# leoelm/Bayesian_inference_for_NN

Measured on NVIDIA B200. Metric: posterior_grad_evals_per_s, higher is better.
Workload: dtype f32 (tensor-core products on two int8 fixed-point slices per operand, kind::i8, exact int32 accumulate; f32 everywhere else)

## Files before the change

### bayesian_inference_for_nn_b200/csrc/tc_fused.cuh

```cuda
#pragma once
#include "tc_layer2.cuh"

namespace pyb {

constexpr int TF_THREADS = 384;
template <int CP> struct TfCfg {
  static constexpr int STAGES = 5;
  static constexpr int W2_BYTES = 2 * 256 * CP * 4;
  static constexpr int ZX_BYTES = 2 * CP * 128 * 4;
  static constexpr int SMEM = STAGES * TP_STAGE_BYTES + 1024  + 1024  + 2048  +
                              128  + W2_BYTES + ZX_BYTES;
  static constexpr int SMEM_I8 = SMEM + 4096;
};
__device__ __forceinline__ void tc_ld_16x256b_x4_raw(uint32_t taddr, uint32_t* r) {
  asm volatile(
      "tcgen05.ld.sync.aligned.16x256b.x4.b32 "
      "{%0, %1, %2, %3, %4, %5, %6, %7, %8, %9, %10, %11, %12, %13, %14, %15}, [%16];"
      : "=r"(r[0]), "=r"(r[1]), "=r"(r[2]), "=r"(r[3]), "=r"(r[4]), "=r"(r[5]), "=r"(r[6]), "=r"(r[7]), "=r"(r[8]),
        "=r"(r[9]), "=r"(r[10]), "=r"(r[11]), "=r"(r[12]), "=r"(r[13]), "=r"(r[14]), "=r"(r[15])
      : "r"(taddr)
      : "memory");
}
__device__ __forceinline__ void tc_mma_i8_pair(uint32_t tmem_d, uint64_t adesc, uint64_t bdesc, uint32_t idesc,
                                               uint32_t accumulate) {
  asm volatile(
      "{\n"
      ".reg .pred p;\n"
      "setp.ne.b32 p, %4, 0;\n"
      "tcgen05.mma.cta_group::2.kind::i8 [%0], %1, %2, %3, p;\n"
      "}\n" ::"r"(tmem_d),
      "l"(adesc), "l"(bdesc), "r"(idesc), "r"(accumulate)
      : "memory");
}
__device__ __forceinline__ void slice4_i8(const float* d, float zq, uint32_t& hw, uint32_t& lw) {
  constexpr float M = 12582912.0f;
  uint32_t hb[4], lb[4];
#pragma unroll
  for (int r = 0; r < 4; ++r) {
    const float t = fmaf(d[r], zq, M);
    const float h = t - M;
    const float e = fmaf(d[r], zq, -h);
    const float u = fmaf(e, 254.0f, M);
    hb[r] = __float_as_uint(t);
    lb[r] = __float_as_uint(u);
  }
  hw = __byte_perm(__byte_perm(hb[0], hb[1], 0x0040), __byte_perm(hb[2], hb[3], 0x0040), 0x5410);
  lw = __byte_perm(__byte_perm(lb[0], lb[1], 0x0040), __byte_perm(lb[2], lb[3], 0x0040), 0x5410);
}

__device__ __forceinline__ void tc_ld_16x256b_x4(uint32_t taddr, float* v) {
  uint32_t r[16];
  asm volatile(
      "tcgen05.ld.sync.aligned.16x256b.x4.b32 "
      "{%0, %1, %2, %3, %4, %5, %6, %7, %8, %9, %10, %11, %12, %13, %14, %15}, [%16];"
      : "=r"(r[0]), "=r"(r[1]), "=r"(r[2]), "=r"(r[3]), "=r"(r[4]), "=r"(r[5]), "=r"(r[6]), "=r"(r[7]), "=r"(r[8]),
        "=r"(r[9]), "=r"(r[10]), "=r"(r[11]), "=r"(r[12]), "=r"(r[13]), "=r"(r[14]), "=r"(r[15])
      : "r"(taddr)
      : "memory");
#pragma unroll
  for (int i = 0; i < 16; ++i) v[i] = __uint_as_float(r[i]);
}
template <int CP>
__device__ __forceinline__ int w2_slot(int h, int c) {
  return ((((h >> 3) * 2 + (h & 1)) * (CP / 4) + (c >> 2)) * 4 + ((h >> 1) & 3)) * 4 + (c & 3);
}
__device__ __forceinline__ void split_pair(float x0, float x1, uint32_t& hw, uint32_t& lw) {
  const __nv_bfloat162 hp = __floats2bfloat162_rn(x0, x1);
  hw = *reinterpret_cast<const uint32_t*>(&hp);
  const __nv_bfloat162 lp = __floats2bfloat162_rn(x0 - __uint_as_float(hw << 16), x1 - __uint_as_float(hw & 0xffff0000u));
  lw = *reinterpret_cast<const uint32_t*>(&lp);
}

template <int CP, bool FWD, int I8 = 0>
__global__ void __cluster_dims__(2, 1, 1) __launch_bounds__(TF_THREADS, 1)
tc_g1_layer2_fused(const __grid_constant__ CUtensorMap tmA_hi, const __grid_constant__ CUtensorMap tmA_lo,
                   const __grid_constant__ CUtensorMap tmB_hi, const __grid_constant__ CUtensorMap tmB_lo,
                   const TcGemmParams p, const Layer2Params l2) {
  constexpr int STAGES = TfCfg<CP>::STAGES;
  extern __shared__ uint8_t smem_raw[];
  uint8_t* smem = smem_raw + ((1024u - (smem_u32(smem_raw) & 1023u)) & 1023u);
  uint8_t* stage_base = smem;
  uint64_t* bars = (uint64_t*)(smem + STAGES * TP_STAGE_BYTES);
  uint64_t* full_bar = bars;
  uint64_t* empty_bar = bars + STAGES;
  uint64_t* tmem_full = bars + 2 * STAGES;
  uint64_t* tmem_empty = bars + 2 * STAGES + 2;
  uint32_t* tmem_ptr = (uint32_t*)(bars + 2 * STAGES + 4);
  float* bias_s = (float*)(smem + STAGES * TP_STAGE_BYTES + 1024);
  float* b2_s = bias_s + 512;
  float* W2_s = b2_s + 32;
  float* zx_s = W2_s + 2 * 256 * CP;
  float* cw_s = zx_s + 2 * CP * 128;
  float* zq_s = cw_s + 512;

  const int warp = __shfl_sync(0xffffffffu, (int)(threadIdx.x >> 5), 0), lane = threadIdx.x & 31;
  const uint32_t rank = cluster_ctarank();
  const int cluster_id = blockIdx.x >> 1, n_clusters = gridDim.x >> 1;
  constexpr int KSTAGE = I8 ? 64 : TC_BK;
  const int nk = (p.K + KSTAGE - 1) / KSTAGE;
  const int H = p.H;
  const int half_rows = H >> 1;
  const uint32_t cta_bytes = 2 * TC_A_TILE_BYTES + 2 * (uint32_t)half_rows * TC_BK * 2;

  if (warp == 8 && lane == 0) {
    asm volatile("prefetch.tensormap [%0];" ::"l"(&tmA_hi) : "memory");
    asm volatile("prefetch.tensormap [%0];" ::"l"(&tmA_lo) : "memory");
    asm volatile("prefetch.tensormap [%0];" ::"l"(&tmB_hi) : "memory");
    asm volatile("prefetch.tensormap [%0];" ::"l"(&tmB_lo) : "memory");
  }
  if (warp == 9 && lane == 0) {
    for (int s = 0; s < STAGES; ++s) { mbar_init(&full_bar[s], 1); mbar_init(&empty_bar[s], 1); }
    mbar_init(&tmem_full[0], 1); mbar_init(&tmem_full[1], 1);
    mbar_init(&tmem_empty[0], 16); mbar_init(&tmem_empty[1], 16);
    asm volatile("fence.mbarrier_init.release.cluster;" ::: "memory");
  }
  if (warp == 10) {
    asm volatile("tcgen05.alloc.cta_group::2.sync.aligned.shared::cta.b32 [%0], %1;" ::"r"(smem_u32(tmem_ptr)), "r"(512)
                 : "memory");
    asm volatile("tcgen05.relinquish_alloc_permit.cta_group::2.sync.aligned;" ::: "memory");
  }
  tc_fence_before();
  __syncthreads();
  cluster_sync_all();
  tc_fence_after();
  const uint32_t tmem_base = *tmem_ptr;

  if (warp >= 8) {
   asm volatile("setmaxnreg.dec.sync.aligned.u32 40;");
   if (warp == 8) {
    if (lane == 0) {
      int stage = 0;
      uint32_t phase = 0;
      for (int item = cluster_id; item < p.total_items; item += n_clusters) {
        int b, mp, split;
        tc_decode(p, item, b, mp, split);
        const int arow = p.a_row0 + (mp * 2 + (int)rank) * 128;
        const int brow = b * H + (int)rank * half_rows;
        for (int kc = 0; kc < nk; ++kc) {
          (I8 ? mbar_wait_sleep(&empty_bar[stage], phase ^ 1) : mbar_wait(&empty_bar[stage], phase ^ 1));
          uint8_t* st = stage_base + stage * TP_STAGE_BYTES;
          if (rank == 0) mbar_expect_tx(&full_bar[stage], 2 * cta_bytes);
          const int k0 = kc * KSTAGE;
          tma_load_2d_pair(st, &tmA_hi, &full_bar[stage], k0, arow);
          tma_load_2d_pair(st + TC_A_TILE_BYTES, &tmA_lo, &full_bar[stage], k0, arow);
          tma_load_2d_pair(st + 2 * TC_A_TILE_BYTES, &tmB_hi, &full_bar[stage], k0, brow);
          tma_load_2d_pair(st + 2 * TC_A_TILE_BYTES + 8192, &tmB_lo, &full_bar[stage], k0, brow);
          if (++stage == STAGES) { stage = 0; phase ^= 1; }
        }
      }
    }
  } else if (warp == 9) {
    if (rank == 0 && lane == 0) {
      const uint32_t idesc = (I8 ? (2u << 4) : (1u << 4)) | (1u << 7) | (1u << 10) | ((uint32_t)(H >> 3) << 17) | ((256u >> 4) << 24);
      int stage = 0, it = 0;
      uint32_t phase = 0;
      const int k_tail = p.K - (nk - 1) * KSTAGE;
      for (int item = cluster_id; item < p.total_items; item += n_clusters, ++it) {
        const int acc = I8 ? 0 : (it & 1);
        const uint32_t acc_phase = I8 ? (uint32_t)(it & 1) : (uint32_t)((it >> 1) & 1);
        (I8 ? mbar_wait_sleep(&tmem_empty[acc], acc_phase ^ 1) : mbar_wait(&tmem_empty[acc], acc_phase ^ 1));
        tc_fence_after();
        const uint32_t d = tmem_base + (uint32_t)acc * 256;
        for (int kc = 0; kc < nk; ++kc) {
          (I8 ? mbar_wait_sleep(&full_bar[stage], phase) : mbar_wait(&full_bar[stage], phase));
          tc_fence_after();
          const uint32_t st = smem_u32(stage_base + stage * TP_STAGE_BYTES);
          const int nks = (kc == nk - 1 && k_tail <= KSTAGE / 2) ? 1 : 2;
          for (int ks = 0; ks < nks; ++ks) {
            const uint32_t koff = ks * 32;
            const uint64_t ah = make_smem_desc_sw64(st + koff);
            const uint64_t al = make_smem_desc_sw64(st + TC_A_TILE_BYTES + koff);
            const uint64_t bh = make_smem_desc_sw64(st + 2 * TC_A_TILE_BYTES + koff);
            const uint64_t bl = make_smem_desc_sw64(st + 2 * TC_A_TILE_BYTES + 8192 + koff);
            const uint32_t accum = (kc != 0) || (ks != 0);
            if (I8) {
              tc_mma_i8_pair(d, ah, bh, idesc, accum);
              tc_mma_i8_pair(d + 256, ah, bl, idesc, accum);
              tc_mma_i8_pair(d + 256, al, bh, idesc, 1);
            } else {
              tc_mma_bf16_pair(d, ah, bh, idesc, accum);
              tc_mma_bf16_pair(d, al, bh, idesc, 1);
              tc_mma_bf16_pair(d, ah, bl, idesc, 1);
            }
          }
          tc_commit_pair(&empty_bar[stage]);
          if (++stage == STAGES) { stage = 0; phase ^= 1; }
        }
        tc_commit_pair(&tmem_full[acc]);
      }
    }
   }
  } else {
    asm volatile("setmaxnreg.inc.sync.aligned.u32 232;");
    const int half = warp >> 2;
    const int quad = warp & 3;
    const int g = lane >> 2, t = lane & 3;
    const int eall = threadIdx.x;
    const uint32_t lane_addr = (uint32_t)(quad * 32) << 16;
    const int Hh = H >> 1;
    const int C = l2.C;
    const float invN = l2.scale / (float)l2.N;
    const int r_own = 2 * (t & 1) + (t >> 1);
    const int row_own = quad * 32 + g + 8 * r_own;
    const int pos0 = quad * 32 + 4 * g;
    const int hbase = half * Hh + 2 * t;
    uint16_t* z2_hi = reinterpret_cast<uint16_t*>(l2.z2_hi);
    uint16_t* z2_lo = reinterpret_cast<uint16_t*>(l2.z2_lo);
    for (int i = eall; i < 2 * 256 * CP; i += 256) W2_s[i] = 0.f;
    if (eall < 32) b2_s[eall] = 0.f;
    asm volatile("bar.sync 1, 256;" ::: "memory");
    auto fetch_consts = [&](int item, int buf) {
      int b, mp, split;
      tc_decode(p, item, b, mp, split);
      const float* th = l2.theta + (int64_t)b * l2.P;
      if (eall < H) {
        const int h = eall;
        const float* src = th + l2.w2_off + (int64_t)h * C;
        const uint32_t dst = smem_u32(W2_s + buf * 256 * CP + w2_slot<CP>(h, 0));
#pragma unroll
        for (int c = 0; c < CP; ++c)
          if (c < C)
            asm volatile("cp.async.ca.shared.global [%0], [%1], 4;" ::"r"(dst + (uint32_t)(((c >> 2) * 16 + (c & 3)) * 4)),
                         "l"(src + c) : "memory");
        asm volatile("cp.async.ca.shared.global [%0], [%1], 4;" ::"r"(smem_u32(bias_s + buf * 256 + h)),
                     "l"(p.bias + (int64_t)b * p.bias_stride + h) : "memory");
      }
      if (eall < C)
        asm volatile("cp.async.ca.shared.global [%0], [%1], 4;" ::"r"(smem_u32(b2_s + buf * 16 + eall)),
                     "l"(th + l2.b2_off + eall) : "memory");
      if (I8 && eall < H) {
        asm volatile("cp.async.ca.shared.global [%0], [%1], 4;" ::"r"(smem_u32(cw_s + buf * 256 + eall)),
                     "l"(l2.cw + (int64_t)b * H + eall) : "memory");
        if (I8 == 2 && !FWD)
          asm volatile("cp.async.ca.shared.global [%0], [%1], 4;" ::"r"(smem_u32(zq_s + buf * 256 + eall)),
                       "l"(l2.zq + (int64_t)b * H + eall) : "memory");
      }
    };
    if (cluster_id < p.total_items) fetch_consts(cluster_id, 0);
    int it = 0;
    for (int item = cluster_id; item < p.total_items; item += n_clusters, ++it) {
      int b, mp, split;
      tc_decode(p, item, b, mp, split);
      const int mt = mp * 2 + (int)rank;
      const int cbuf = it & 1;
      const int acc = I8 ? 0 : cbuf;
      const uint32_t acc_phase = I8 ? (uint32_t)(it & 1) : (uint32_t)((it >> 1) & 1);
      float* bs = bias_s + cbuf * 256;
      float* b2b = b2_s + cbuf * 16;
      float* W2b = W2_s + cbuf * 256 * CP;
      float sxr[4] = {0.f, 0.f, 0.f, 0.f};
      if (I8) {
#pragma unroll
        for (int r = 0; r < 4; ++r) {
          const int rg = mt * 128 + quad * 32 + g + 8 * r;
          sxr[r] = rg < p.M_valid ? __ldg(l2.sx + rg) : 0.f;
        }
      }
      asm volatile("cp.async.wait_all;" ::: "memory");
      asm volatile("bar.sync 1, 256;" ::: "memory");
      (I8 ? mbar_wait_sleep(&tmem_full[acc], acc_phase) : mbar_wait(&tmem_full[acc], acc_phase));
      tc_fence_after();
      const int64_t blk_w = (((((int64_t)b * p.out_tiles + mt) * H) + hbase) * 128 + pos0) >> 2;
      uint2* pa_hi = reinterpret_cast<uint2*>(p.out_hi) + blk_w;
      uint2* pa_lo = reinterpret_cast<uint2*>(p.out_lo) + blk_w;
      uint2* pz_hi = reinterpret_cast<uint2*>(l2.zt_hi) + blk_w;
      uint2* pz_lo = reinterpret_cast<uint2*>(l2.zt_lo) + blk_w;
      const float4* w4b = reinterpret_cast<const float4*>(W2b) + (((half * Hh) >> 3) * 2 * (CP / 4)) * 4 + t;
      const float* bsb = bs + hbase;
      const float* cwb = cw_s + cbuf * 256 + hbase;
      const float* zqb = zq_s + cbuf * 256 + hbase;
      uint32_t* pzi_hi = nullptr; uint32_t* pzi_lo = nullptr;
      if (I8 == 2 && !FWD) {
        const int64_t blk_b = ((((int64_t)b * p.out_tiles + mt) * H) + hbase) * 128 + pos0;
        pzi_hi = reinterpret_cast<uint32_t*>(l2.zi_hi + blk_b);
        pzi_lo = reinterpret_cast<uint32_t*>(l2.zi_lo + blk_b);
      }
      float2 z[4][CP / 2];
#pragma unroll
      for (int r = 0; r < 4; ++r)
#pragma unroll
        for (int c = 0; c < CP / 2; ++c) z[r][c] = make_float2(0.f, 0.f);
      uint32_t mask[4] = {0u, 0u, 0u, 0u};
#pragma unroll
      for (int ch = 0; ch < 4; ++ch) {
        if (ch * 32 < Hh) {
          const uint32_t col = (uint32_t)(acc * 256 + half * Hh + ch * 32);
          float v[32];
          if (I8) {
#pragma unroll
            for (int hf = 0; hf < 2; ++hf) {
              uint32_t rh[16], rc[16];
              tc_ld_16x256b_x4_raw(tmem_base + lane_addr + ((uint32_t)(16 * hf) << 16) + col, rh);
              tc_ld_16x256b_x4_raw(tmem_base + lane_addr + ((uint32_t)(16 * hf) << 16) + 256u + col, rc);
              asm volatile("tcgen05.wait::ld.sync.aligned;" ::: "memory");
#pragma unroll
              for (int j = 0; j < 16; ++j)
                v[16 * hf + j] = fmaf((float)(int)rc[j], 1.0f / 254.0f, (float)(int)rh[j]);
            }
          } else {
            tc_ld_16x256b_x4(tmem_base + lane_addr + col, v);
            tc_ld_16x256b_x4(tmem_base + lane_addr + (16u << 16) + col, v + 16);
            asm volatile("tcgen05.wait::ld.sync.aligned;" ::: "memory");
          }
          uint32_t m = 0u;
#pragma unroll
          for (int kb = 0; kb < 4; ++kb) {
            const float2 bb = *reinterpret_cast<const float2*>(bsb + ch * 32 + 8 * kb);
            float2 cc = make_float2(0.f, 0.f);
            if (I8) cc = *reinterpret_cast<const float2*>(cwb + ch * 32 + 8 * kb);
            float a[4][2];
#pragma unroll
            for (int r = 0; r < 4; ++r) {
              const float* vv = v + (r >> 1) * 16 + kb * 4 + (r & 1) * 2;
              if (I8) {
                a[r][0] = fmaxf(fmaf(vv[0], sxr[r] * cc.x, bb.x), 0.f);
                a[r][1] = fmaxf(fmaf(vv[1], sxr[r] * cc.y, bb.y), 0.f);
              } else {
                a[r][0] = fmaxf(vv[0] + bb.x, 0.f);
                a[r][1] = fmaxf(vv[1] + bb.y, 0.f);
              }
              if (!FWD) {
                m |= (a[r][0] > 0.f ? 1u : 0u) << (kb * 8 + r * 2);
                m |= (a[r][1] > 0.f ? 1u : 0u) << (kb * 8 + r * 2 + 1);
              }
            }
#pragma unroll
            for (int i = 0; i < 2; ++i) {
              const float4* w4 = w4b + (((ch * 4 + kb) * 2 + i) * (CP / 4)) * 4;
#pragma unroll
              for (int c4 = 0; c4 < CP / 4; ++c4) {
                const float4 w = w4[c4 * 4];
                const float2 w01 = make_float2(w.x, w.y), w23 = make_float2(w.z, w.w);
#pragma unroll
                for (int r = 0; r < 4; ++r) {
                  const float2 aa = make_float2(a[r][i], a[r][i]);
                  z[r][2 * c4] = __ffma2_rn(aa, w01, z[r][2 * c4]);
                  z[r][2 * c4 + 1] = __ffma2_rn(aa, w23, z[r][2 * c4 + 1]);
                }
              }
              if (!FWD) {
                uint32_t hw0, lw0, hw1, lw1;
                split_pair(a[0][i], a[1][i], hw0, lw0);
                split_pair(a[2][i], a[3][i], hw1, lw1);
                const int w_off = (ch * 32 + 8 * kb + i) * 32;
                __stcs(pa_hi + w_off, make_uint2(hw0, hw1));
                __stcs(pa_lo + w_off, make_uint2(lw0, lw1));
              }
            }
          }
          mask[ch] = m;
        }
      }
      tc_fence_before();
      __syncwarp();
      if (lane == 0) mbar_arrive_leader_relaxed(&tmem_empty[acc]);
      if (item + n_clusters < p.total_items) fetch_consts(item + n_clusters, cbuf ^ 1);
      float zo[CP];
      {
        const bool b0 = t & 1, b1 = t & 2;
#pragma unroll
        for (int c = 0; c < CP; ++c) {
          const float z0 = (c & 1) ? z[0][c >> 1].y : z[0][c >> 1].x, z1 = (c & 1) ? z[1][c >> 1].y : z[1][c >> 1].x;
          const float z2v = (c & 1) ? z[2][c >> 1].y : z[2][c >> 1].x, z3 = (c & 1) ? z[3][c >> 1].y : z[3][c >> 1].x;
          float k0 = b0 ? z2v : z0, k1 = b0 ? z3 : z1;
          const float g0 = __shfl_xor_sync(0xffffffffu, b0 ? z0 : z2v, 1);
          const float g1 = __shfl_xor_sync(0xffffffffu, b0 ? z1 : z3, 1);
          k0 = b0 ? g0 + k0 : k0 + g0;
          k1 = b0 ? g1 + k1 : k1 + g1;
          const float kk = b1 ? k1 : k0;
          const float gg = __shfl_xor_sync(0xffffffffu, b1 ? k0 : k1, 2);
          zo[c] = b1 ? gg + kk : kk + gg;
        }
      }
#pragma unroll
      for (int c = 0; c < CP; ++c) zx_s[(half * CP + c) * 128 + row_own] = zo[c];
      asm volatile("bar.sync 2, 256;" ::: "memory");
      float zf[CP], dz[CP];
#pragma unroll
      for (int c = 0; c < CP; ++c) zf[c] = (b2b[c] + zx_s[c * 128 + row_own]) + zx_s[(CP + c) * 128 + row_own];
      const int row_g = mt * 128 + row_own;
      if (FWD) {
        if (half == 0 && row_g < p.M_valid) {
          float* o = l2.fwd_out + ((int64_t)b * l2.N + row_g) * C;
          if (l2.out_act == PYB_ACT_SOFTMAX) {
            float mx = -INFINITY;
#pragma unroll
            for (int c = 0; c < CP; ++c) if (c < C) mx = fmaxf(mx, zf[c]);
            float se = 0.f;
#pragma unroll
            for (int c = 0; c < CP; ++c) if (c < C) se += expf(zf[c] - mx);
            const float inv = 1.0f / se;
#pragma unroll
            for (int c = 0; c < CP; ++c) if (c < C) o[c] = expf(zf[c] - mx) * inv;
          } else {
#pragma unroll
            for (int c = 0; c < CP; ++c) if (c < C) o[c] = act_apply(zf[c], l2.out_act);
          }
        }
        continue;
      }
      float loss_r = 0.f;
      l2_loss_dz<CP>(l2, row_g, row_g < p.M_valid, zf, dz, loss_r, invN);
      if (half == 0) {
        const int64_t blk2 = (((int64_t)b * p.out_tiles + mt) * L2_CMAX) * 128 + pos0 + r_own;
#pragma unroll
        for (int c = 0; c < CP; ++c) {
          __nv_bfloat16 hb, lb;
          split_bf16(dz[c], hb, lb);
          z2_hi[blk2 + c * 128] = __bfloat16_as_ushort(hb);
          z2_lo[blk2 + c * 128] = __bfloat16_as_ushort(lb);
        }
        const int64_t grp = (int64_t)b * l2.n_groups + mt * 4 + quad;
        float mine = 0.f;
#pragma unroll
        for (int c = 0; c < CP; ++c) {
          const float sm = warp_sum(dz[c]);
          if (lane == c) mine = sm;
        }
        if (lane < CP) l2.b2_partial[grp * L2_CMAX + lane] = mine;
        const float ls = warp_sum(loss_r);
        if (lane == 0) l2.loss_partial[grp] = (double)ls;
      }
      float2 dzp[4][CP / 2];
#pragma unroll
      for (int r = 0; r < 4; ++r) {
        const int src = (lane & ~3) | ((r >> 1) | ((r & 1) << 1));
#pragma unroll
        for (int c = 0; c < CP / 2; ++c) {
          dzp[r][c].x = __shfl_sync(0xffffffffu, dz[2 * c], src);
          dzp[r][c].y = __shfl_sync(0xffffffffu, dz[2 * c + 1], src);
        }
      }
#pragma unroll
      for (int ch = 0; ch < 4; ++ch) {
        if (ch * 32 < Hh) {
          const uint32_t m = mask[ch];
#pragma unroll
          for (int kb = 0; kb < 4; ++kb) {
#pragma unroll
            for (int i = 0; i < 2; ++i) {
              const float4* w4 = w4b + (((ch * 4 + kb) * 2 + i) * (CP / 4)) * 4;
              float2 s[4];
#pragma unroll
              for (int r = 0; r < 4; ++r) s[r] = make_float2(0.f, 0.f);
#pragma unroll
              for (int c4 = 0; c4 < CP / 4; ++c4) {
                const float4 w = w4[c4 * 4];
                const float2 w01 = make_float2(w.x, w.y), w23 = make_float2(w.z, w.w);
#pragma unroll
                for (int r = 0; r < 4; ++r) {
                  s[r] = __ffma2_rn(dzp[r][2 * c4], w01, s[r]);
                  s[r] = __ffma2_rn(dzp[r][2 * c4 + 1], w23, s[r]);
                }
              }
              float d[4];
#pragma unroll
              for (int r = 0; r < 4; ++r) d[r] = ((m >> (kb * 8 + r * 2 + i)) & 1u) ? s[r].x + s[r].y : 0.f;
              const int w_off = (ch * 32 + 8 * kb + i) * 32;
              if (I8 == 2) {
                uint32_t hw, lw;
                slice4_i8(d, zqb[ch * 32 + 8 * kb + i], hw, lw);
                __stcs(pzi_hi + w_off, hw);
                __stcs(pzi_lo + w_off, lw);
              } else {
                uint32_t hw0, lw0, hw1, lw1;
                split_pair(d[0], d[1], hw0, lw0);
                split_pair(d[2], d[3], hw1, lw1);
                __stcs(pz_hi + w_off, make_uint2(hw0, hw1));
                __stcs(pz_lo + w_off, make_uint2(lw0, lw1));
              }
            }
          }
        }
      }
    }
  }
  tc_fence_before();
  __syncthreads();
  cluster_sync_all();
  if (warp == 10) {
    tc_fence_after();
    asm volatile("tcgen05.dealloc.cta_group::2.sync.aligned.b32 %0, %1;" ::"r"(tmem_base), "r"(512) : "memory");
  }
}

}
```

### bayesian_inference_for_nn_b200/csrc/tc_layer2.cuh

```cuda
#pragma once
#include "tc_gemm.cuh"

namespace pyb {

__device__ __forceinline__ void split_bf16(float x, __nv_bfloat16& hi, __nv_bfloat16& lo) {
  hi = __float2bfloat16_rn(x);
  lo = __float2bfloat16_rn(x - __bfloat162float(hi));
}

__global__ void k_split_rows(const float* src, int64_t R, int C, int64_t lds, __nv_bfloat16* hi, __nv_bfloat16* lo,
                             int64_t ldd) {
  const int64_t total = R * C;
  for (int64_t i = (int64_t)blockIdx.x * blockDim.x + threadIdx.x; i < total; i += (int64_t)gridDim.x * blockDim.x) {
    int64_t r = i / C;
    int c = (int)(i - r * C);
    __nv_bfloat16 h, l;
    split_bf16(src[r * lds + c], h, l);
    hi[r * ldd + c] = h;
    lo[r * ldd + c] = l;
  }
}
__global__ void k_split_rows2(const float* __restrict__ src, int64_t R, int C2, int64_t lds, __nv_bfloat16* __restrict__ hi,
                              __nv_bfloat16* __restrict__ lo, int64_t ldd) {
  const int64_t total = R * C2;
  for (int64_t i = (int64_t)blockIdx.x * blockDim.x + threadIdx.x; i < total; i += (int64_t)gridDim.x * blockDim.x) {
    const int64_t r = i / C2;
    const int c = 2 * (int)(i - r * C2);
    const float2 v = *reinterpret_cast<const float2*>(src + r * lds + c);
    __nv_bfloat16 h0, l0, h1, l1;
    split_bf16(v.x, h0, l0);
    split_bf16(v.y, h1, l1);
    *reinterpret_cast<__nv_bfloat162*>(hi + r * ldd + c) = __nv_bfloat162(h0, h1);
    *reinterpret_cast<__nv_bfloat162*>(lo + r * ldd + c) = __nv_bfloat162(l0, l1);
  }
}

__host__ __device__ __forceinline__ int fused_row_pos(int r) { return (r & ~31) | ((r & 7) << 2) | ((r >> 3) & 3); }

__global__ void k_split_transpose(const float* src, int64_t sb, int R, int C, int64_t lds, __nv_bfloat16* hi,
                                  __nv_bfloat16* lo, int64_t db, int64_t ldd, int perm = 0) {
  __shared__ float t[32][33];
  const float* s = src + (int64_t)blockIdx.z * sb;
  int c0 = blockIdx.x * 32, r0 = blockIdx.y * 32;
  for (int i = threadIdx.y; i < 32; i += 8) {
    int r = r0 + i, c = c0 + threadIdx.x;
    t[i][threadIdx.x] = (r < R && c < C) ? s[(int64_t)r * lds + c] : 0.f;
  }
  __syncthreads();
  for (int i = threadIdx.y; i < 32; i += 8) {
    int c = c0 + i, r = r0 + threadIdx.x;
    if (c < C && r < R) {
      __nv_bfloat16 h, l;
      split_bf16(t[threadIdx.x][i], h, l);
      int64_t o = (int64_t)blockIdx.z * db + (int64_t)c * ldd + (perm ? fused_row_pos(r) : r);
      hi[o] = h;
      lo[o] = l;
    }
  }
}

__global__ void k_fill_ones_perm(__nv_bfloat16* p, int n) {
  for (int i = blockIdx.x * blockDim.x + threadIdx.x; i < n; i += gridDim.x * blockDim.x)
    p[fused_row_pos(i)] = __float2bfloat16_rn(1.0f);
}
__global__ void k_fill_bf16(__nv_bfloat16* p, int64_t n, float v) {
  for (int64_t i = (int64_t)blockIdx.x * blockDim.x + threadIdx.x; i < n; i += (int64_t)gridDim.x * blockDim.x)
    p[i] = __float2bfloat16_rn(v);
}

constexpr int L2_CMAX = 16;
constexpr int L2_ROWS = 256;
struct Layer2Params {
  const __nv_bfloat16* a_hi; const __nv_bfloat16* a_lo;
  __nv_bfloat16* zt_hi; __nv_bfloat16* zt_lo;
  __nv_bfloat16* z2_hi; __nv_bfloat16* z2_lo;
  int k_tiles;
  const float* theta; int64_t P; int64_t w2_off, b2_off;
  int H, C, N, act1, out_act, loss_kind;
  const int32_t* y_i; const float* y_f;
  float scale;
  double* loss_partial;
  float* b2_partial;
  int n_groups, n_tiles;
  float* fwd_out;
  const float* sx;
  const float* cw;
  const float* zq;
  int8_t* zi_hi; int8_t* zi_lo;
  int dbg_flags;
  unsigned long long* dbg;
};
__device__ __forceinline__ float2 unpack_bf16x2(uint32_t v) {
  return make_float2(__uint_as_float(v << 16), __uint_as_float(v & 0xffff0000u));
}
__device__ __forceinline__ uint32_t pack_bf16x2(__nv_bfloat16 a, __nv_bfloat16 b) {
  return (uint32_t)__bfloat16_as_ushort(a) | ((uint32_t)__bfloat16_as_ushort(b) << 16);
}
template <int CP, typename LT>
__device__ __forceinline__ void l2_loss_dz(const Layer2Params& p, int r, bool valid, const float* z, float* dz,
                                           LT& loss_acc, float invN) {
  const int C = p.C;
#pragma unroll
  for (int c = 0; c < CP; ++c) dz[c] = 0.f;
  if (!valid) return;
  if (p.loss_kind == PYB_LOSS_SPARSE_CE) {
    float mx = -INFINITY;
#pragma unroll
    for (int c = 0; c < CP; ++c) if (c < C) mx = fmaxf(mx, z[c]);
    float se = 0.f;
#pragma unroll
    for (int c = 0; c < CP; ++c) if (c < C) se += expf(z[c] - mx);
    const int yi = p.y_i[r];
    float zy = 0.f;
#pragma unroll
    for (int c = 0; c < CP; ++c) if (c == yi) zy = z[c];
    loss_acc += (LT)(logf(se) - (zy - mx));
    const float inv = 1.0f / se;
#pragma unroll
    for (int c = 0; c < CP; ++c)
      if (c < C) dz[c] = (expf(z[c] - mx) * inv - (c == yi ? 1.f : 0.f)) * invN;
  } else {
    float acc = 0.f;
    const float sc = 2.0f * invN / (float)C;
#pragma unroll
    for (int c = 0; c < CP; ++c)
      if (c < C) {
        float a = act_apply(z[c], p.out_act);
        float df = a - p.y_f[(int64_t)r * C + c];
        acc += df * df;
        dz[c] = sc * df * act_grad_from_output(a, p.out_act);
      }
    loss_acc += (LT)(acc / (float)C);
  }
}
template <int CP>
__global__ void __launch_bounds__(128, 4) k_layer2(Layer2Params p) {
  __shared__ __align__(16) float W2s[256 * CP];
  __shared__ float b2s[CP];
  __shared__ uint32_t mask_s[2][8][128];
  __shared__ float redf[4][CP];
  __shared__ double scratch[32];
  const int t = threadIdx.x, b = blockIdx.y;
  const int H = p.H, C = p.C;
  const float* th = p.theta + (int64_t)b * p.P;
  for (int i = t; i < H * CP; i += 128) {
    int h = i / CP, c = i % CP;
    W2s[i] = (c < C) ? th[p.w2_off + (int64_t)h * C + c] : 0.f;
  }
  if (t < CP) b2s[t] = (t < C) ? th[p.b2_off + t] : 0.f;
  __syncthreads();
  const uint32_t* ah = reinterpret_cast<const uint32_t*>(p.a_hi);
  const uint32_t* al = reinterpret_cast<const uint32_t*>(p.a_lo);
  uint32_t* zh = reinterpret_cast<uint32_t*>(p.zt_hi);
  uint32_t* zl = reinterpret_cast<uint32_t*>(p.zt_lo);
  uint32_t* z2h = reinterpret_cast<uint32_t*>(p.z2_hi);
  uint32_t* z2l = reinterpret_cast<uint32_t*>(p.z2_lo);
  const int64_t ld2 = 64;
  float accb[CP];
#pragma unroll
  for (int c = 0; c < CP; ++c) accb[c] = 0.f;
  double loss_acc = 0.0;
  const float invN = p.scale / (float)p.N;
  const bool relu = p.act1 == PYB_ACT_RELU;
  const int nhb = (H + 31) >> 5;
  for (int tile = blockIdx.x; tile < p.n_tiles; tile += gridDim.x) {
    const int r0 = tile * L2_ROWS + 2 * t;
    const int64_t tile128 = (int64_t)b * p.k_tiles + tile * 2 + (t >> 6);
    const int64_t col = tile128 * H * 64 + (t & 63);
    const int64_t col2 = tile128 * L2_CMAX * 64 + (t & 63);
    const bool v0 = r0 < p.N, v1 = r0 + 1 < p.N;
    float z0[CP], z1[CP];
#pragma unroll
    for (int c = 0; c < CP; ++c) { z0[c] = b2s[c]; z1[c] = b2s[c]; }
    for (int hb = 0; hb < nhb; ++hb) {
      uint32_t m0 = 0u, m1 = 0u;
      const uint32_t* ahp = ah + (int64_t)(hb * 32) * ld2 + col;
      const uint32_t* alp = al + (int64_t)(hb * 32) * ld2 + col;
      const int jn = min(32, H - hb * 32);
#pragma unroll 4
      for (int j = 0; j < jn; ++j) {
        const float2 hi = unpack_bf16x2(ahp[(int64_t)j * ld2]);
        const float2 lo = unpack_bf16x2(alp[(int64_t)j * ld2]);
        const float a0 = hi.x + lo.x, a1v = hi.y + lo.y;
        m0 |= (a0 > 0.f ? 1u : 0u) << j;
        m1 |= (a1v > 0.f ? 1u : 0u) << j;
        const float4* w = reinterpret_cast<const float4*>(&W2s[(hb * 32 + j) * CP]);
#pragma unroll
        for (int q4 = 0; q4 < CP / 4; ++q4) {
          const float4 wv = w[q4];
          z0[q4 * 4 + 0] = fmaf(a0, wv.x, z0[q4 * 4 + 0]); z1[q4 * 4 + 0] = fmaf(a1v, wv.x, z1[q4 * 4 + 0]);
          z0[q4 * 4 + 1] = fmaf(a0, wv.y, z0[q4 * 4 + 1]); z1[q4 * 4 + 1] = fmaf(a1v, wv.y, z1[q4 * 4 + 1]);
          z0[q4 * 4 + 2] = fmaf(a0, wv.z, z0[q4 * 4 + 2]); z1[q4 * 4 + 2] = fmaf(a1v, wv.z, z1[q4 * 4 + 2]);
          z0[q4 * 4 + 3] = fmaf(a0, wv.w, z0[q4 * 4 + 3]); z1[q4 * 4 + 3] = fmaf(a1v, wv.w, z1[q4 * 4 + 3]);
        }
      }
      mask_s[0][hb][t] = m0;
      mask_s[1][hb][t] = m1;
    }
    float dz0[CP], dz1[CP];
    l2_loss_dz<CP>(p, r0, v0, z0, dz0, loss_acc, invN);
    l2_loss_dz<CP>(p, r0 + 1, v1, z1, dz1, loss_acc, invN);
#pragma unroll
    for (int c = 0; c < CP; ++c) {
      accb[c] += dz0[c] + dz1[c];
      __nv_bfloat16 h0, l0, h1, l1;
      split_bf16(dz0[c], h0, l0);
      split_bf16(dz1[c], h1, l1);
      z2h[(int64_t)c * ld2 + col2] = pack_bf16x2(h0, h1);
      z2l[(int64_t)c * ld2 + col2] = pack_bf16x2(l0, l1);
    }
    for (int hb = 0; hb < nhb; ++hb) {
      const uint32_t m0 = mask_s[0][hb][t], m1 = mask_s[1][hb][t];
      uint32_t* zhp = zh + (int64_t)(hb * 32) * ld2 + col;
      uint32_t* zlp = zl + (int64_t)(hb * 32) * ld2 + col;
      const int jn = min(32, H - hb * 32);
#pragma unroll 4
// ... 161 lines not shown
```

### bayesian_inference_for_nn_b200/csrc/tc_path.cu

```cuda
#include <cstdlib>
#include <cstring>
#include "tc_fused_mma.cuh"
#include <algorithm>

namespace pyb {

typedef CUresult (*PFN_encodeTiled)(CUtensorMap*, CUtensorMapDataType, cuuint32_t, void*, const cuuint64_t*,
                                    const cuuint64_t*, const cuuint32_t*, const cuuint32_t*, CUtensorMapInterleave,
                                    CUtensorMapSwizzle, CUtensorMapL2promotion, CUtensorMapFloatOOBfill);
static PFN_encodeTiled get_encode() {
  static PFN_encodeTiled fn = nullptr;
  if (!fn) {
    void* f = nullptr;
    cudaDriverEntryPointQueryResult q;
    PYB_CUDA(cudaGetDriverEntryPoint("cuTensorMapEncodeTiled", &f, cudaEnableDefault, &q));
    PYB_REQUIRE(f != nullptr && q == cudaDriverEntryPointSuccess, PYB_ERR_CUDA, "cuTensorMapEncodeTiled unavailable");
    fn = (PFN_encodeTiled)f;
  }
  return fn;
}
static CUtensorMap make_map_blocked(const void* base, int64_t blocks, int rows_per_block, int box_rows) {
  CUtensorMap m;
  cuuint64_t dims[3] = {128, (cuuint64_t)rows_per_block, (cuuint64_t)blocks};
  cuuint64_t strides[2] = {256, (cuuint64_t)rows_per_block * 256};
// ... 97 lines not shown
  if (h->tc) ((TcState*)h->tc)->train.ready = false;
}
void tc_invalidate_track(pyb_handle* h) {
  if (h->tc) ((TcState*)h->tc)->track.ready = false;
}

bool tc_supported_rows(pyb_handle* h, int64_t n_rows) {
  const Model& m = h->model;
  if (m.n_layers != 2) return false;
  const LayerDesc& L1 = m.layer[0];
  const LayerDesc& L2 = m.layer[1];
  if (!L1.use_bias || !L2.use_bias) return false;
  if (L1.fan_out % 16 != 0 || L1.fan_out < 16 || L1.fan_out > 256) return false;
  if (L1.fan_in % 8 != 0 || L1.fan_in < 64) return false;
  if (L2.fan_out > L2_CMAX) return false;
  if (L1.act == PYB_ACT_SOFTMAX) return false;
  return n_rows >= 128;
}
bool tc_supported(pyb_handle* h, int64_t S) {
  (void)S;
  return h->have_data && tc_supported_rows(h, h->N);
}

template <int EPI, int ACT>
static void launch_gemm_inst(pyb_handle* h, int grid, const CUtensorMap& a_hi, const CUtensorMap& a_lo,
                             const CUtensorMap& b_hi, const CUtensorMap& b_lo, const TcGemmParams& p) {
  PYB_CUDA(cudaFuncSetAttribute(tc_gemm_bf16x3<EPI, ACT>, cudaFuncAttributeMaxDynamicSharedMemorySize, TC_SMEM_BYTES));
  tc_gemm_bf16x3<EPI, ACT><<<grid, TC_THREADS, TC_SMEM_BYTES, h->stream>>>(a_hi, a_lo, b_hi, b_lo, p);
}
template <int EPI, int ACT>
static void launch_pair_inst(pyb_handle* h, int grid, const CUtensorMap& a_hi, const CUtensorMap& a_lo,
                             const CUtensorMap& b_hi, const CUtensorMap& b_lo, const TcGemmParams& p) {
  PYB_CUDA(cudaFuncSetAttribute(tc_gemm_pair_bf16x3<EPI, ACT>, cudaFuncAttributeMaxDynamicSharedMemorySize, TP_SMEM_BYTES));
  tc_gemm_pair_bf16x3<EPI, ACT><<<grid, TP_THREADS, TP_SMEM_BYTES, h->stream>>>(a_hi, a_lo, b_hi, b_lo, p);
}
static bool pair_ok(const pyb_handle* h, const TcGemmParams& p) {
  if (!h->opt_tc_pair || p.b_blocked || p.H < 32 || p.n_mtiles < 2) return false;
  if (p.n_btiles > 0) return p.a_blocked && p.n_mtiles == 2 && (p.H % 16) == 0;
  if ((p.H % 32) != 0) return false;
  return !p.a_blocked && p.a_batch_rows == 0;
}
static void launch_gemm_tc(pyb_handle* h, const CUtensorMap& a_hi, const CUtensorMap& a_lo,
                           const CUtensorMap& b_hi, const CUtensorMap& b_lo, TcGemmParams p, double flops,
                           const CUtensorMap* bp_hi = nullptr, const CUtensorMap* bp_lo = nullptr) {
  if (p.k_splits <= 1) { p.k_splits = 1; p.chunks_per_split = (p.K + TC_BK - 1) / TC_BK; p.split_stride = 0; }
  p.vec_store = p.epi == EPI_STORE && ((uintptr_t)p.out % 16 == 0) && (p.out_stride % 4 == 0) && (p.out_ld % 4 == 0) &&
                (p.split_stride % 4 == 0);
  int grid = std::min(p.total_items, h->sm_count);
  prof_begin(h);
  if (bp_hi && bp_lo && pair_ok(h, p) && p.n_btiles > 1 && p.epi == EPI_STORE && p.transpose_out && h->opt_tc_dual &&
      p.H <= 256 && (p.H / 2) * TC_BK * 2 <= 8192) {
    p.total_items = p.n_batch * p.k_splits * ((p.n_btiles + 1) / 2);
    grid = std::min(2 * p.total_items, (h->sm_count / 2) * 2);
    PYB_CUDA(cudaFuncSetAttribute(tc_gemm_pair_dual_bf16x3, cudaFuncAttributeMaxDynamicSharedMemorySize, TD_SMEM_BYTES));
    tc_gemm_pair_dual_bf16x3<<<grid, TP_THREADS, TD_SMEM_BYTES, h->stream>>>(a_hi, a_lo, *bp_hi, *bp_lo, p);
    prof_end(h, flops);
    count_launch(h);
    return;
  }
  if (bp_hi && bp_lo && pair_ok(h, p)) {
    grid = std::min(2 * p.total_items, (h->sm_count / 2) * 2);
    if (p.epi == EPI_STORE) launch_pair_inst<EPI_STORE, 0>(h, grid, a_hi, a_lo, *bp_hi, *bp_lo, p);
    else if (p.act == PYB_ACT_RELU) launch_pair_inst<EPI_BIAS_ACT_T_SPLIT, PYB_ACT_RELU>(h, grid, a_hi, a_lo, *bp_hi, *bp_lo, p);
    else if (p.act == PYB_ACT_TANH) launch_pair_inst<EPI_BIAS_ACT_T_SPLIT, PYB_ACT_TANH>(h, grid, a_hi, a_lo, *bp_hi, *bp_lo, p);
    else if (p.act == PYB_ACT_SIGMOID) launch_pair_inst<EPI_BIAS_ACT_T_SPLIT, PYB_ACT_SIGMOID>(h, grid, a_hi, a_lo, *bp_hi, *bp_lo, p);
    else launch_pair_inst<EPI_BIAS_ACT_T_SPLIT, PYB_ACT_LINEAR>(h, grid, a_hi, a_lo, *bp_hi, *bp_lo, p);
    prof_end(h, flops);
    count_launch(h);
    return;
  }
  if (p.epi == EPI_STORE) launch_gemm_inst<EPI_STORE, 0>(h, grid, a_hi, a_lo, b_hi, b_lo, p);
  else if (p.act == PYB_ACT_RELU) launch_gemm_inst<EPI_BIAS_ACT_T_SPLIT, PYB_ACT_RELU>(h, grid, a_hi, a_lo, b_hi, b_lo, p);
  else if (p.act == PYB_ACT_TANH) launch_gemm_inst<EPI_BIAS_ACT_T_SPLIT, PYB_ACT_TANH>(h, grid, a_hi, a_lo, b_hi, b_lo, p);
  else if (p.act == PYB_ACT_SIGMOID) launch_gemm_inst<EPI_BIAS_ACT_T_SPLIT, PYB_ACT_SIGMOID>(h, grid, a_hi, a_lo, b_hi, b_lo, p);
  else launch_gemm_inst<EPI_BIAS_ACT_T_SPLIT, PYB_ACT_LINEAR>(h, grid, a_hi, a_lo, b_hi, b_lo, p);
  prof_end(h, flops);
  count_launch(h);
}


template <int CP, bool FWD, int I8>
static void launch_fused_i8(pyb_handle* h, int grid, const CUtensorMap& a_hi, const CUtensorMap& a_lo,
                            const CUtensorMap& b_hi, const CUtensorMap& b_lo, const TcGemmParams& p, const Layer2Params& l2) {
  PYB_CUDA(cudaFuncSetAttribute(tc_g1_layer2_fused<CP, FWD, I8>, cudaFuncAttributeMaxDynamicSharedMemorySize, TfCfg<CP>::SMEM_I8));
  tc_g1_layer2_fused<CP, FWD, I8><<<grid, TF_THREADS, TfCfg<CP>::SMEM_I8, h->stream>>>(a_hi, a_lo, b_hi, b_lo, p, l2);
}
template <int CP>
static void launch_fused_inst(pyb_handle* h, int grid, const CUtensorMap& a_hi, const CUtensorMap& a_lo,
                              const CUtensorMap& b_hi, const CUtensorMap& b_lo, const TcGemmParams& p, const Layer2Params& l2,
                              int i8 = 0) {
  if (i8 && !l2.fwd_out && h->opt_tc_epi_mma) {
    if (i8 >= 2) {
      PYB_CUDA(cudaFuncSetAttribute(tc_fused_i8_mma<CP, true>, cudaFuncAttributeMaxDynamicSharedMemorySize, TfmCfg::SMEM));
      tc_fused_i8_mma<CP, true><<<grid, TFM_THREADS, TfmCfg::SMEM, h->stream>>>(a_hi, a_lo, b_hi, b_lo, p, l2);
    } else {
      PYB_CUDA(cudaFuncSetAttribute(tc_fused_i8_mma<CP, false>, cudaFuncAttributeMaxDynamicSharedMemorySize, TfmCfg::SMEM));
      tc_fused_i8_mma<CP, false><<<grid, TFM_THREADS, TfmCfg::SMEM, h->stream>>>(a_hi, a_lo, b_hi, b_lo, p, l2);
    }
    return;
  }
  if (i8) {
    if (l2.fwd_out) launch_fused_i8<CP, true, 1>(h, grid, a_hi, a_lo, b_hi, b_lo, p, l2);
    else if (i8 >= 2) launch_fused_i8<CP, false, 2>(h, grid, a_hi, a_lo, b_hi, b_lo, p, l2);
    else launch_fused_i8<CP, false, 1>(h, grid, a_hi, a_lo, b_hi, b_lo, p, l2);
    return;
  }
  if (l2.fwd_out) {
    PYB_CUDA(cudaFuncSetAttribute(tc_g1_layer2_fused<CP, true>, cudaFuncAttributeMaxDynamicSharedMemorySize, TfCfg<CP>::SMEM));
    tc_g1_layer2_fused<CP, true><<<grid, TF_THREADS, TfCfg<CP>::SMEM, h->stream>>>(a_hi, a_lo, b_hi, b_lo, p, l2);
    return;
  }
  PYB_CUDA(cudaFuncSetAttribute(tc_g1_layer2_fused<CP, false>, cudaFuncAttributeMaxDynamicSharedMemorySize, TfCfg<CP>::SMEM));
  tc_g1_layer2_fused<CP, false><<<grid, TF_THREADS, TfCfg<CP>::SMEM, h->stream>>>(a_hi, a_lo, b_hi, b_lo, p, l2);
}
static bool fused_ok(const pyb_handle* h, int H, int act1) {
  return h->opt_tc_pair && h->opt_tc_fuse && act1 == PYB_ACT_RELU && (H == 128 || H == 256);
}

static int i8_mode(const pyb_handle* h, bool backward, bool resident) {
  const Model& m = h->model;
  int want = h->opt_tc_i8;
  if (want < 0) want = (resident && backward && h->i8_guard_ok) ? 2 : 0;
  if (want <= 0 || !fused_ok(h, m.layer[0].fan_out, m.layer[0].act) || m.layer[1].fan_out > L2_CMAX) return 0;
  if (m.layer[0].fan_in > 32768) return 0;
  if (!backward) return 1;
  const bool ce = h->loss_kind == PYB_LOSS_SPARSE_CE && m.layer[1].act == PYB_ACT_SOFTMAX;
  return (want >= 2 && ce && m.layer[0].fan_out == 256) ? 2 : 1;
}

static void tc_prepare_data_i8(pyb_handle* h, TcData& d, const float* X, int64_t N, int mode) {
  const int D = d.D;
  const int64_t Npad = d.Npad;
  d.Dk = (D + 15) / 16 * 16;
  d.col_mean.alloc(D); d.col_absmax.alloc(D); d.sx.alloc(N); d.sf.alloc(D + 1);
  d.xs_hi.alloc(N * d.Dk); d.xs_lo.alloc(N * d.Dk);
  d.stat_sum.alloc((size_t)I8_STAT_CHUNKS * D); d.stat_max.alloc((size_t)I8_STAT_CHUNKS * D);
  k_col_stats<<<dim3((D + 31) / 32, I8_STAT_CHUNKS), dim3(32, 32), 0, h->stream>>>(X, N, D, d.stat_sum.p, d.stat_max.p);
  k_col_stats_final<<<(D + 255) / 256, 256, 0, h->stream>>>(d.stat_sum.p, d.stat_max.p, I8_STAT_CHUNKS, N, D, d.col_mean.p,
                                                           d.col_absmax.p);
  count_launch(h);
  const int wpb = 8;
  k_slice_x_rows_i8<<<(unsigned)std::min<int64_t>((N + wpb - 1) / wpb, 8 * (int64_t)h->sm_count), wpb * 32, 0, h->stream>>>(
      X, N, D, d.col_mean.p, d.xs_hi.p, d.xs_lo.p, d.sx.p, d.Dk);
  count_launch(h, 2);
  d.mXs_hi = make_map_u8p(d.xs_hi.p, d.Dk, N, d.Dk, 128);
  d.mXs_lo = make_map_u8p(d.xs_lo.p, d.Dk, N, d.Dk, 128);
  if (mode >= 2) {
    d.xts_hi.alloc((int64_t)(D + 1) * Npad); d.xts_lo.alloc((int64_t)(D + 1) * Npad);
    PYB_CUDA(cudaMemsetAsync(d.xts_hi.p, 0, (size_t)(D + 1) * Npad, h->stream));
    PYB_CUDA(cudaMemsetAsync(d.xts_lo.p, 0, (size_t)(D + 1) * Npad, h->stream));
    dim3 g2((D + 31) / 32, (unsigned)((N + 31) / 32), 1), blk(32, 8);
    k_slice_xt_i8<<<g2, blk, 0, h->stream>>>(X, N, D, d.col_absmax.p, d.xts_hi.p, d.xts_lo.p, Npad);
    k_xt_i8_tail<<<(unsigned)((std::max<int64_t>(N, D + 1) + 255) / 256), 256, 0, h->stream>>>(
        d.xts_hi.p + (int64_t)D * Npad, N, d.col_absmax.p, d.sf.p, D);
    count_launch(h, 2);
    const int n_t = (D + 1 + 255) / 256, Ht = (((D + 1 + n_t - 1) / n_t) + 15) / 16 * 16;
    d.mXTs_hi = make_map_u8p(d.xts_hi.p, Npad, D + 1, Npad, Ht / 2);
    d.mXTs_lo = make_map_u8p(d.xts_lo.p, Npad, D + 1, Npad, Ht / 2);
  }
  d.i8 = mode;
}

static void tc_prepare_data(pyb_handle* h, TcData& d, const float* X, int64_t N, bool need_xt, bool resident = false) {
  const Model& m = h->model;
  const int D = m.layer[0].fan_in;
  d.N = N; d.D = D;
// ... 472 lines not shown
```

Before: 10950.

## Release TMEM earlier, prefetch labels, fuse b2/loss reductions, add timing probes

```diff
diff --git a/bayesian_inference_for_nn_b200/csrc/tc_fused.cuh b/bayesian_inference_for_nn_b200/csrc/tc_fused.cuh
--- a/bayesian_inference_for_nn_b200/csrc/tc_fused.cuh
+++ b/bayesian_inference_for_nn_b200/csrc/tc_fused.cuh
@@ -71,7 +71,30 @@
   lw = *reinterpret_cast<const uint32_t*>(&lp);
 }
 
-template <int CP, bool FWD, int I8 = 0>
+template <int NV>
+__device__ __forceinline__ float warp_sum_scatter16(const float* v, int lane) {
+  const bool u16 = lane & 16, u8 = lane & 8, u4 = lane & 4, u2 = lane & 2;
+  float a[8], b[4], c[2];
+#pragma unroll
+  for (int j = 0; j < 8; ++j) {
+    const float lo = j < NV ? v[j < NV ? j : 0] : 0.f, hi = j + 8 < NV ? v[j + 8 < NV ? j + 8 : 0] : 0.f;
+    a[j] = (u16 ? hi : lo) + __shfl_xor_sync(0xffffffffu, u16 ? lo : hi, 16);
+  }
+#pragma unroll
+  for (int j = 0; j < 4; ++j) b[j] = (u8 ? a[j + 4] : a[j]) + __shfl_xor_sync(0xffffffffu, u8 ? a[j] : a[j + 4], 8);
+#pragma unroll
+  for (int j = 0; j < 2; ++j) c[j] = (u4 ? b[j + 2] : b[j]) + __shfl_xor_sync(0xffffffffu, u4 ? b[j] : b[j + 2], 4);
+  const float d = (u2 ? c[1] : c[0]) + __shfl_xor_sync(0xffffffffu, u2 ? c[0] : c[1], 2);
+  return d + __shfl_xor_sync(0xffffffffu, d, 1);
+}
+
+template <bool TL>
+__device__ __forceinline__ long long tl_clock() {
+  if constexpr (TL) return clock64();
+  else return 0;
+}
+
+template <int CP, bool FWD, int I8 = 0, bool TL = false>
 __global__ void __cluster_dims__(2, 1, 1) __launch_bounds__(TF_THREADS, 1)
 tc_g1_layer2_fused(const __grid_constant__ CUtensorMap tmA_hi, const __grid_constant__ CUtensorMap tmA_lo,
                    const __grid_constant__ CUtensorMap tmB_hi, const __grid_constant__ CUtensorMap tmB_lo,
@@ -155,15 +178,21 @@
       int stage = 0, it = 0;
       uint32_t phase = 0;
       const int k_tail = p.K - (nk - 1) * KSTAGE;
+      long long t_wait = 0, t_loop = 0, t_fill = 0;
       for (int item = cluster_id; item < p.total_items; item += n_clusters, ++it) {
         const int acc = I8 ? 0 : (it & 1);
         const uint32_t acc_phase = I8 ? (uint32_t)(it & 1) : (uint32_t)((it >> 1) & 1);
+        const long long c0 = tl_clock<TL>();
         (I8 ? mbar_wait_sleep(&tmem_empty[acc], acc_phase ^ 1) : mbar_wait(&tmem_empty[acc], acc_phase ^ 1));
         tc_fence_after();
+        const long long c1 = tl_clock<TL>();
+        t_wait += c1 - c0;
         const uint32_t d = tmem_base + (uint32_t)acc * 256;
         for (int kc = 0; kc < nk; ++kc) {
+          const long long f0 = tl_clock<TL>();
           (I8 ? mbar_wait_sleep(&full_bar[stage], phase) : mbar_wait(&full_bar[stage], phase));
           tc_fence_after();
+          t_fill += tl_clock<TL>() - f0;
           const uint32_t st = smem_u32(stage_base + stage * TP_STAGE_BYTES);
           const int nks = (kc == nk - 1 && k_tail <= KSTAGE / 2) ? 1 : 2;
           for (int ks = 0; ks < nks; ++ks) {
@@ -187,6 +216,13 @@
           if (++stage == STAGES) { stage = 0; phase ^= 1; }
         }
         tc_commit_pair(&tmem_full[acc]);
+        t_loop += tl_clock<TL>() - c1;
+      }
+      if (TL) {
+        l2.dbg[blockIdx.x * 8 + 0] = (unsigned long long)t_wait;
+        l2.dbg[blockIdx.x * 8 + 1] = (unsigned long long)t_loop;
+        l2.dbg[blockIdx.x * 8 + 2] = (unsigned long long)t_fill;
+        l2.dbg[blockIdx.x * 8 + 3] = (unsigned long long)it;
       }
     }
    }
@@ -237,8 +273,11 @@
       }
     };
     if (cluster_id < p.total_items) fetch_consts(cluster_id, 0);
+    const bool ce = l2.loss_kind == PYB_LOSS_SPARSE_CE;
     int it = 0;
+    long long e_top = 0, e_wait = 0, e_A = 0, e_x = 0, e_sm = 0, e_B = 0;
     for (int item = cluster_id; item < p.total_items; item += n_clusters, ++it) {
+      const long long s0 = tl_clock<TL>();
       int b, mp, split;
       tc_decode(p, item, b, mp, split);
       const int mt = mp * 2 + (int)rank;
@@ -256,10 +295,15 @@
           sxr[r] = rg < p.M_valid ? __ldg(l2.sx + rg) : 0.f;
         }
       }
+      const int row_g = mt * 128 + row_own;
+      const bool valid = row_g < p.M_valid;
+      const int yi = (!FWD && ce && valid) ? __ldg(l2.y_i + row_g) : 0;
       asm volatile("cp.async.wait_all;" ::: "memory");
       asm volatile("bar.sync 1, 256;" ::: "memory");
+      const long long s1 = tl_clock<TL>();
       (I8 ? mbar_wait_sleep(&tmem_full[acc], acc_phase) : mbar_wait(&tmem_full[acc], acc_phase));
       tc_fence_after();
+      const long long s2 = tl_clock<TL>();
       const int64_t blk_w = (((((int64_t)b * p.out_tiles + mt) * H) + hbase) * 128 + pos0) >> 2;
       uint2* pa_hi = reinterpret_cast<uint2*>(p.out_hi) + blk_w;
       uint2* pa_lo = reinterpret_cast<uint2*>(p.out_lo) + blk_w;
@@ -301,6 +345,11 @@
             tc_ld_16x256b_x4(tmem_base + lane_addr + col, v);
             tc_ld_16x256b_x4(tmem_base + lane_addr + (16u << 16) + col, v + 16);
             asm volatile("tcgen05.wait::ld.sync.aligned;" ::: "memory");
+          }
+          if ((ch + 1) * 32 >= Hh) {
+            tc_fence_before();
+            __syncwarp();
+            if (lane == 0) mbar_arrive_leader_relaxed(&tmem_empty[acc]);
           }
           uint32_t m = 0u;
 #pragma unroll
@@ -351,10 +400,12 @@
           mask[ch] = m;
         }
       }
-      tc_fence_before();
-      __syncwarp();
-      if (lane == 0) mbar_arrive_leader_relaxed(&tmem_empty[acc]);
+      const long long s3 = tl_clock<TL>();
       if (item + n_clusters < p.total_items) fetch_consts(item + n_clusters, cbuf ^ 1);
+      float yf[CP];
+#pragma unroll
+      for (int c = 0; c < CP; ++c)
+        yf[c] = (!FWD && !ce && c < C && valid) ? __ldg(l2.y_f + (int64_t)row_g * C + c) : 0.f;
       float zo[CP];
       {
         const bool b0 = t & 1, b1 = t & 2;
@@ -375,12 +426,12 @@
 #pragma unroll
       for (int c = 0; c < CP; ++c) zx_s[(half * CP + c) * 128 + row_own] = zo[c];
       asm volatile("bar.sync 2, 256;" ::: "memory");
-      float zf[CP], dz[CP];
-#pragma unroll
-      for (int c = 0; c < CP; ++c) zf[c] = (b2b[c] + zx_s[c * 128 + row_own]) + zx_s[(CP + c) * 128 + row_own];
-      const int row_g = mt * 128 + row_own;
+      const long long s4 = tl_clock<TL>();
       if (FWD) {
-        if (half == 0 && row_g < p.M_valid) {
+        if (half == 0 && valid) {
+          float zf[CP];
+#pragma unroll
+          for (int c = 0; c < CP; ++c) zf[c] = (b2b[c] + zx_s[c * 128 + row_own]) + zx_s[(CP + c) * 128 + row_own];
           float* o = l2.fwd_out + ((int64_t)b * l2.N + row_g) * C;
           if (l2.out_act == PYB_ACT_SOFTMAX) {
             float mx = -INFINITY;
@@ -399,8 +450,11 @@
         }
         continue;
       }
+      float zf[CP], dz[CP];
+#pragma unroll
+      for (int c = 0; c < CP; ++c) zf[c] = (b2b[c] + zx_s[c * 128 + row_own]) + zx_s[(CP + c) * 128 + row_own];
       float loss_r = 0.f;
-      l2_loss_dz<CP>(l2, row_g, row_g < p.M_valid, zf, dz, loss_r, invN);
+      l2_loss_dz_y<CP>(l2, valid, yi, yf, zf, dz, loss_r, invN);
       if (half == 0) {
         const int64_t blk2 = (((int64_t)b * p.out_tiles + mt) * L2_CMAX) * 128 + pos0 + r_own;
 #pragma unroll
@@ -411,15 +465,18 @@
           z2_lo[blk2 + c * 128] = __bfloat16_as_ushort(lb);
         }
         const int64_t grp = (int64_t)b * l2.n_groups + mt * 4 + quad;
-        float mine = 0.f;
-#pragma unroll
-        for (int c = 0; c < CP; ++c) {
-          const float sm = warp_sum(dz[c]);
-          if (lane == c) mine = sm;
-        }
-        if (lane < CP) l2.b2_partial[grp * L2_CMAX + lane] = mine;
-        const float ls = warp_sum(loss_r);
-        if (lane == 0) l2.loss_partial[grp] = (double)ls;
+        constexpr int NV = CP < 16 ? CP + 1 : 16;
+        float v[NV];
+#pragma unroll
+        for (int c = 0; c < NV; ++c) v[c] = c < CP ? dz[c < CP ? c : 0] : loss_r;
+        const float sm = warp_sum_scatter16<NV>(v, lane);
+        if (!(lane & 1) && (lane >> 1) < CP) l2.b2_partial[grp * L2_CMAX + (lane >> 1)] = sm;
+        if (CP < 16) {
+          if (lane == 2 * CP) l2.loss_partial[grp] = (double)sm;
+        } else {
+          const float ls = warp_sum(loss_r);
+          if (lane == 0) l2.loss_partial[grp] = (double)ls;
+        }
       }
       float2 dzp[4][CP / 2];
 #pragma unroll
@@ -431,6 +488,7 @@
           dzp[r][c].y = __shfl_sync(0xffffffffu, dz[2 * c + 1], src);
         }
       }
+      const long long s5 = tl_clock<TL>();
 #pragma unroll
       for (int ch = 0; ch < 4; ++ch) {
         if (ch * 32 < Hh) {
@@ -473,6 +531,17 @@
           }
         }
       }
+      e_top += s1 - s0; e_wait += s2 - s1; e_A += s3 - s2; e_x += s4 - s3; e_sm += s5 - s4; e_B += tl_clock<TL>() - s5;
+    }
+    if (TL && warp == 0 && lane == 0) {
+      if (blockIdx.x & 1) {
+        l2.dbg[blockIdx.x * 8 + 0] = (unsigned long long)e_x;
+        l2.dbg[blockIdx.x * 8 + 1] = (unsigned long long)e_sm;
+      }
+      l2.dbg[blockIdx.x * 8 + 4] = (unsigned long long)e_top;
+      l2.dbg[blockIdx.x * 8 + 5] = (unsigned long long)e_wait;
+      l2.dbg[blockIdx.x * 8 + 6] = (unsigned long long)e_A;
+      l2.dbg[blockIdx.x * 8 + 7] = (unsigned long long)e_B;
     }
   }
   tc_fence_before();
diff --git a/bayesian_inference_for_nn_b200/csrc/tc_layer2.cuh b/bayesian_inference_for_nn_b200/csrc/tc_layer2.cuh
--- a/bayesian_inference_for_nn_b200/csrc/tc_layer2.cuh
+++ b/bayesian_inference_for_nn_b200/csrc/tc_layer2.cuh
@@ -97,8 +97,8 @@
   return (uint32_t)__bfloat16_as_ushort(a) | ((uint32_t)__bfloat16_as_ushort(b) << 16);
 }
 template <int CP, typename LT>
-__device__ __forceinline__ void l2_loss_dz(const Layer2Params& p, int r, bool valid, const float* z, float* dz,
-                                           LT& loss_acc, float invN) {
+__device__ __forceinline__ void l2_loss_dz_y(const Layer2Params& p, bool valid, int yi, const float* yf, const float* z,
+                                             float* dz, LT& loss_acc, float invN) {
   const int C = p.C;
 #pragma unroll
   for (int c = 0; c < CP; ++c) dz[c] = 0.f;
@@ -109,8 +109,7 @@
     for (int c = 0; c < CP; ++c) if (c < C) mx = fmaxf(mx, z[c]);
     float se = 0.f;
 #pragma unroll
-    for (int c = 0; c < CP; ++c) if (c < C) se += expf(z[c] - mx);
-    const int yi = p.y_i[r];
+    for (int c = 0; c < CP; ++c) if (c < C) { dz[c] = expf(z[c] - mx); se += dz[c]; }
     float zy = 0.f;
 #pragma unroll
     for (int c = 0; c < CP; ++c) if (c == yi) zy = z[c];
@@ -118,7 +117,7 @@
     const float inv = 1.0f / se;
 #pragma unroll
     for (int c = 0; c < CP; ++c)
-      if (c < C) dz[c] = (expf(z[c] - mx) * inv - (c == yi ? 1.f : 0.f)) * invN;
+      if (c < C) dz[c] = (dz[c] * inv - (c == yi ? 1.f : 0.f)) * invN;
   } else {
     float acc = 0.f;
     const float sc = 2.0f * invN / (float)C;
@@ -126,12 +125,18 @@
     for (int c = 0; c < CP; ++c)
       if (c < C) {
         float a = act_apply(z[c], p.out_act);
-        float df = a - p.y_f[(int64_t)r * C + c];
+        float df = a - yf[c];
         acc += df * df;
         dz[c] = sc * df * act_grad_from_output(a, p.out_act);
       }
     loss_acc += (LT)(acc / (float)C);
   }
+}
+template <int CP, typename LT>
+__device__ __forceinline__ void l2_loss_dz(const Layer2Params& p, int r, bool valid, const float* z, float* dz,
+                                           LT& loss_acc, float invN) {
+  const bool ce = p.loss_kind == PYB_LOSS_SPARSE_CE;
+  l2_loss_dz_y<CP>(p, valid, (valid && ce) ? p.y_i[r] : 0, ce ? nullptr : p.y_f + (int64_t)r * p.C, z, dz, loss_acc, invN);
 }
 template <int CP>
 __global__ void __launch_bounds__(128, 4) k_layer2(Layer2Params p) {
diff --git a/bayesian_inference_for_nn_b200/csrc/tc_path.cu b/bayesian_inference_for_nn_b200/csrc/tc_path.cu
--- a/bayesian_inference_for_nn_b200/csrc/tc_path.cu
+++ b/bayesian_inference_for_nn_b200/csrc/tc_path.cu
@@ -203,6 +203,14 @@
 template <int CP, bool FWD, int I8>
 static void launch_fused_i8(pyb_handle* h, int grid, const CUtensorMap& a_hi, const CUtensorMap& a_lo,
                             const CUtensorMap& b_hi, const CUtensorMap& b_lo, const TcGemmParams& p, const Layer2Params& l2) {
+  if constexpr (!FWD && I8 == 2) {
+    if (l2.dbg) {
+      PYB_CUDA(cudaFuncSetAttribute(tc_g1_layer2_fused<CP, false, 2, true>, cudaFuncAttributeMaxDynamicSharedMemorySize,
+                                    TfCfg<CP>::SMEM_I8));
+      tc_g1_layer2_fused<CP, false, 2, true><<<grid, TF_THREADS, TfCfg<CP>::SMEM_I8, h->stream>>>(a_hi, a_lo, b_hi, b_lo, p, l2);
+      return;
+    }
+  }
   PYB_CUDA(cudaFuncSetAttribute(tc_g1_layer2_fused<CP, FWD, I8>, cudaFuncAttributeMaxDynamicSharedMemorySize, TfCfg<CP>::SMEM_I8));
   tc_g1_layer2_fused<CP, FWD, I8><<<grid, TF_THREADS, TfCfg<CP>::SMEM_I8, h->stream>>>(a_hi, a_lo, b_hi, b_lo, p, l2);
 }
```

Result: faster. 11080, median of 6 (+1.2%).
